# Illumina/Pisces

Measured on AMD Instinct MI355X. Metric: candidate loci/s at 500x depth, higher is better.
Workload: dtype int32 counts + f64 likelihoods; 1 GPU; BASELINE config 2: synthetic 100000 loci x 500x amplicon pileup, SNV-only, gVCF, per GPU per step; device-resident packed tuples; depth=500, ring_batches=6, tile_loci=56, parallelism=interval-shard x1

## Files before the change

### pisces_amd/build.py

```python
import os
import shutil
import subprocess

HERE = os.path.dirname(os.path.abspath(__file__))
CSRC = os.path.join(HERE, "csrc")
LIB = os.path.join(HERE, "libpisceship.so")
SOURCES = ["pisces_hip.hip", "expander.cpp", "finder.cpp", "vcf_format.cpp", "diploid.cpp"]
HEADERS = ["kernels.hip.h", "stream_kernels.hip.h", "store_kernels.hip.h", "surface_store.inc.h", "finder_kernels.hip.h", "bgzf_kernels.hip.h", "bam_kernels.hip.h", "device_math.hip.h", "surface_reads.inc.h", "surface_flush.inc.h", "surface_device.inc.h", "surface_bam.inc.h", "surface_comm.inc.h", "expander.h", "read_walk.h", "finder.h", "finder_walk.h", "diploid.h", "genotype_core.h", os.path.join("..", "..", "include", "pisces_hip.h")]


def hipcc_path():
    for cand in (shutil.which("hipcc"), "/opt/rocm/bin/hipcc"):
        if cand and os.path.exists(cand):
            return cand
    raise RuntimeError("hipcc not found (need ROCm: /opt/rocm/bin/hipcc)")


def is_stale():
    if not os.path.exists(LIB):
        return True
    t = os.path.getmtime(LIB)
    return any(os.path.getmtime(os.path.join(CSRC, f)) > t for f in SOURCES + HEADERS)


def source_hash():
    import hashlib
    hsh = hashlib.sha1()
    for f in sorted(SOURCES + HEADERS):
        with open(os.path.join(CSRC, f), "rb") as fp:
            hsh.update(f.encode() + b"\0" + fp.read())
    return hsh.hexdigest()


LAST_BUILD = {"mode": None, "seconds": 0.0}


def build_native(force=False, verbose=False, extra_flags=(), out=None):
    import time
    lib = LIB if out is None else out
    if out is None and not force and not is_stale():
        LAST_BUILD.update(mode="reused", seconds=0.0)
        return lib
    t0 = time.time()
    tmp = f"{lib}.{os.getpid()}.tmp"
    cmd = [hipcc_path(), "--offload-arch=gfx950", "-O3", "-std=c++17", "-fPIC", "-shared", "-ffp-contract=off",
           "-fno-fast-math", "-Wall", "-Wno-unused-function", "-x", "hip",
           *extra_flags, *[os.path.join(CSRC, s) for s in SOURCES], "-lpthread", "-ldl", "-o", tmp]
    if verbose:
        print(" ".join(cmd))
    subprocess.check_call(cmd)
    os.replace(tmp, lib)
    if out is None:
        LAST_BUILD.update(mode="rebuilt", seconds=time.time() - t0)
    return lib


if __name__ == "__main__":
    import sys
    build_native(force="--force" in sys.argv, verbose=True)
    print(LIB)
```

### pisces_amd/csrc/kernels.hip.h

```cpp
#pragma once
#include <hip/hip_runtime.h>
#include <stdint.h>

#include "device_math.hip.h"
#include "genotype_core.h"

namespace pisces {

constexpr int kBlock = 256;
constexpr int kTile = 64;
constexpr int kFolded = 18;
constexpr int kUnroll = 8;
constexpr int kSlotsPerTile = 4 * kTile;
#ifndef PISCES_TOTAL_SHARDS
#define PISCES_TOTAL_SHARDS 64
#endif
constexpr int kTotalShards = PISCES_TOTAL_SHARDS;
constexpr int kTotalStride = 16;
constexpr int kRefMargin = 32;
constexpr int kRefWin = kTile + 2 * kRefMargin;
constexpr int kWaveRows = 32;
constexpr int kWaveRow = kTile;
constexpr int kWaveRegion = kWaveRows * kWaveRow;
constexpr int kQLutLds = 128;
// ... 39 lines not shown
        u32x4 v[kUnroll];
#pragma unroll
        for (int u = 0; u < kUnroll; u++) {
            int64_t j = i + (int64_t)u * kBlock;
            v[u] = j < n4 ? __builtin_nontemporal_load(&p4[j]) : (u32x4){~0u, ~0u, ~0u, ~0u};
        }
#pragma unroll
        for (int u = 0; u < kUnroll; u++) {
            op(v[u].x); op(v[u].y); op(v[u].z); op(v[u].w);
        }
    }
    for (int64_t i = aend + tid; i < end; i += kBlock) op(tuples[i]);
}

__device__ __forceinline__ void copy_record(PiscesCalledAllele* dst, const PiscesCalledAllele* src)
{
    const unsigned long long sb = (unsigned long long)__double_as_longlong(src->strand_bias_score);
    uint4* dp = reinterpret_cast<uint4*>(dst);
    dp[0] = make_uint4((uint32_t)src->position, (uint32_t)src->total_coverage, (uint32_t)src->allele_support, (uint32_t)src->reference_support);
    dp[1] = make_uint4((uint32_t)src->num_no_calls, (uint32_t)src->coverage_by_dir[0], (uint32_t)src->coverage_by_dir[1], (uint32_t)src->coverage_by_dir[2]);
    dp[2] = make_uint4((uint32_t)src->support_by_dir[0], (uint32_t)src->support_by_dir[1], (uint32_t)src->support_by_dir[2], (uint32_t)src->variant_qscore);
    dp[3] = make_uint4((uint32_t)sb, (uint32_t)(sb >> 32), (uint32_t)(uint16_t)src->genotype_qscore | ((uint32_t)(uint16_t)src->noise_level << 16), (uint32_t)src->filter_bits | ((uint32_t)src->info << 16));
}

struct PointCounts {
    int cov[3], sup[3];
    int total, nocalls, refsup, support;
};

struct HistBlock {
    static __device__ __forceinline__ int idx(int a, int d, int l) { return (a * 3 + d) * kTile + l; }
};
struct HistWave {
    static __device__ __forceinline__ int idx(int a, int d, int l) { return (a * 4 + d) * kWaveRow + (int)PISCES_TUPLE_COLUMN(l, d); }
};

struct HistLinear {
    static __device__ __forceinline__ int idx(int a, int d, int l) { return (a * 4 + d) * kWaveRow + l; }
};

struct LocusCounts { int h[6][3]; };

template <typename H = HistBlock>
__device__ __forceinline__ LocusCounts load_counts(const int* hist, int l)
{
    LocusCounts lc;
// ... 342 lines not shown
__device__ __forceinline__ void stream_tuples_wave(const uint32_t* __restrict__ tuples, int64_t begin, int64_t end, int lane, int wid,
                                                   Op op, Pre pre)
{
    int64_t abegin = (begin + 3) & ~(int64_t)3;
    int64_t aend = end & ~(int64_t)3;
    if (abegin > aend) { abegin = end; aend = end; }
    const int tid = wid * 64 + lane;
    const u32x4* __restrict__ p4 = reinterpret_cast<const u32x4*>(tuples + abegin);
    const uint32_t n4 = (uint32_t)((aend - abegin) >> 2);
    constexpr uint32_t kBatch = 64u * kWaveUnroll;
    const uint32_t nb = (uint32_t)__builtin_amdgcn_readfirstlane((int)((n4 + kBatch - 1) / kBatch));
    u32x4 cur[kWaveUnroll], nxt[kWaveUnroll];
    auto load = [&](u32x4* v, uint32_t b) {
#pragma unroll
        for (int u = 0; u < kWaveUnroll; u++) {
            const uint32_t j = min(b * kBatch + (uint32_t)u * 64u + (uint32_t)lane, n4 - 1u);
            v[u] = __builtin_nontemporal_load(&p4[j]);
        }
    };
    auto consume = [&](const u32x4* v) {
#pragma unroll
        for (int u = 0; u < kWaveUnroll; u++) { op(v[u].x); op(v[u].y); op(v[u].z); op(v[u].w); }
    };
    const bool streams = (uint32_t)wid < nb;
    if (NW == 2) {
        if (streams) load(cur, (uint32_t)__builtin_amdgcn_readfirstlane(wid));
        __builtin_amdgcn_sched_barrier(0);
        pre();
    } else {
        pre();
        if (streams) load(cur, (uint32_t)__builtin_amdgcn_readfirstlane(wid));
    }
    for (int64_t i = begin + tid; i < abegin; i += 64 * NW) op(tuples[i]);
    if (streams) {
        uint32_t b = (uint32_t)__builtin_amdgcn_readfirstlane(wid);
        const uint32_t m = (nb - b + NW - 1) / NW;
        for (uint32_t p = (m - 1) / 2; p > 0; p--) {
            load(nxt, b + NW);
            __builtin_amdgcn_sched_barrier(0);
            consume(cur);
            __builtin_amdgcn_sched_barrier(0);
            load(cur, b + 2 * NW);
            __builtin_amdgcn_sched_barrier(0);
            consume(nxt);
            __builtin_amdgcn_sched_barrier(0);
            b += 2 * NW;
        }
        if (((m - 1) & 1u) != 0) {
            load(nxt, b + NW);
            __builtin_amdgcn_sched_barrier(0);
            consume(cur);
            __builtin_amdgcn_sched_barrier(0);
#pragma unroll
            for (int u = 0; u < kWaveUnroll; u++) cur[u] = nxt[u];
            b += NW;
        }
        if (b == nb - 1 && (n4 % kBatch)) {
#pragma unroll
            for (int u = 0; u < kWaveUnroll; u++)
                if (b * kBatch + (uint32_t)u * 64u + (uint32_t)lane >= n4) cur[u] = (u32x4){~0u, ~0u, ~0u, ~0u};
        }
        consume(cur);
    }
    for (int64_t i = aend + tid; i < end; i += 64 * NW) op(tuples[i]);
}

__device__ __forceinline__ void wave_lds_sync()
{
    __builtin_amdgcn_fence(__ATOMIC_SEQ_CST, "workgroup");
    __builtin_amdgcn_wave_barrier();
}

template <typename H = HistWave>
__device__ __forceinline__ uint32_t slow_alleles(const int* hist, const uint8_t* s_refwin, uint32_t slow, int l, int pos, int rt, int ref_rank,
                                                 const uint8_t* __restrict__ ref, int64_t win_lo, int64_t win_hi, PiscesCalledAllele* slots,
                                                 const DeviceParams& P)
{
    uint32_t called = 0;
    const int ref_a = (rt < 4) ? rt : PISCES_ALLELE_N;
#pragma unroll 1
    for (int k = 0; k < 5; k++) {
        if (!((slow >> k) & 1u)) continue;
        const bool isRef = k == 4;
        const int a = isRef ? ref_a : allele_of_rank(k);
        const LocusCounts lc = load_counts_wave<H>(hist, l);
        const PointCounts c = point_counts_of(lc, a, isRef, rt, 0);
        int vq = 0;
        if (c.support > 0 && c.total != 0) vq = poisson_qscore_out_of_line(c.support, c.total, P.err_q, P.max_vq, P.ln10);
        if (!isRef && vq < P.min_vq) continue;
        SbResult sb = {0.0, 0, 0, 0};
        if (c.support > 0) sb = strand_bias_out_of_line(c.cov, c.sup, P);
        PiscesCalledAllele r;
        (void)finish_allele<false>(c, pos, a, isRef, rt, vq, sb, ref, win_lo, win_hi, P, r, s_refwin, kRefMargin + l);
        copy_record(&slots[isRef ? ref_rank : k], &r);
        if (!isRef) called |= 1u << k;
    }
    return called;
}

template <int NW, typename H = HistWave>
__device__ __forceinline__ void call_phase_wave(const int* hist, const uint8_t* s_refwin, uint8_t* s_vmask, const PiscesTile& tile, const int t,
                                                const int l, const int wid, const uint8_t* __restrict__ ref, const int32_t ref_start,
                                                const int64_t ref_len, PiscesCalledAllele* __restrict__ records,
                                                PiscesTileResult* __restrict__ tile_results, const DeviceParams& P
#ifdef PISCES_TIMING
                                                , const long long tc0, const long long tc1
#endif
                                                )
{
    const int pos = tile.start_position + l;
    const uint8_t refb = s_refwin[kRefMargin + l];
    const bool in_ref = l < tile.n_loci && refb != 0;
    const int rt = in_ref ? allele_type_of_base(refb) : PISCES_ALLELE_N;
    const int64_t win_lo = (int64_t)ref_start - 1, win_hi = win_lo + ref_len;
    auto slot_of = [&](int k) { return records + ((int64_t)t * kSlotsPerTile + l * 4 + k); };
    const bool dirty = locus_is_dirty(P, pos);
    const LocusCounts lc = load_counts_wave<H>(hist, l);
    const bool ref_wave = wid == 0, var_wave = wid == NW - 1;
    if (P.folded_out && ref_wave && l < tile.n_loci) {
        const unsigned rel = (unsigned)(pos - P.folded_first);
        if (rel < (unsigned)P.folded_n) {
            int32_t* const dst = P.folded_out + (size_t)rel * PISCES_FOLDED_PER_LOCUS;
#pragma unroll
            for (int a = 0; a < 6; a++)
#pragma unroll
                for (int d = 0; d < 3; d++) dst[a * 3 + d] = lc.h[a][d];
        }
    }

    const bool tabs = tables_complete(P);
    auto fast_allele = [&](const PointCounts& c, int a, bool isRef, PiscesCalledAllele& rec) -> bool {
        int vq = 0;
        double sb_score = 0.0;
        int sb_ok = 0, sb_var = 0, sb_cov = 0;
        if (!tabs) return false;
        const AlleleTables tb = request_allele_tables(isRef, c.support, c.total, c.refsup, c.cov, c.sup, P);
        if (c.support > 0 && c.total != 0 && !poisson_qscore_try(c.support, c.total, P, tb, vq)) return false;
        if (!isRef && vq < P.min_vq) return true;
        if (c.support > 0 && !strand_bias_try(c.cov, c.sup, P, tb, sb_score, sb_ok, sb_var, sb_cov)) return false;
        const GqPre g = {tb.gq_idx, tb.gq_cap};
        const SbResult sb = {sb_score, sb_ok, sb_var, sb_cov};
        if (!finish_allele<true>(c, pos, a, isRef, rt, vq, sb, ref, win_lo, win_hi, P, rec, s_refwin, kRefMargin + l, nullptr, &g)) return false;
        return true;
    };
    bool ref_emitted = false;
    int ref_rank = 0;
    uint32_t slow = 0;
    uint32_t vmask = 0;
    const int ref_a = (rt < 4) ? rt : PISCES_ALLELE_N;
    if (ref_wave) {
        const PointCounts c = point_counts_of(lc, ref_a, true, rt, 0);
        if (in_ref && P.include_ref && !P.variants_only && (P.emit_zero_cov || c.total + c.nocalls > 0)) {
            ref_rank = (rt < 4) ? rank_of_allele(rt) : 0;
            ref_emitted = true;
            PiscesCalledAllele rec;
            if (fast_allele(c, ref_a, true, rec)) copy_record(slot_of(ref_rank), &rec);
            else slow |= 16u;
        }
    }
#ifdef PISCES_TIMING
    const long long tcA = wall_clock64();
#endif
    if (var_wave && in_ref && rt < 4 && !P.refs_only && !dirty) {
#pragma unroll 1
        for (int k = 0; k < 4; k++) {
            const int a = allele_of_rank(k);
            if (a == rt) continue;
            const PointCounts c = point_counts_of(lc, a, false, rt, 0);
            if (c.support == 0) continue;
            if (!variant_passes_frequency(c, P)) continue;
            PiscesCalledAllele r;
            r.position = 0;
            if (!fast_allele(c, a, false, r)) { slow |= 1u << k; continue; }
            if (r.position == 0) continue;
            copy_record(slot_of(k), &r);
            vmask |= 1u << k;
        }
    }
    if (__builtin_expect(__ballot(slow != 0) != 0ull, 0))
        vmask |= slow_alleles<H>(hist, s_refwin, slow, l, pos, rt, ref_rank, ref, win_lo, win_hi, records + ((int64_t)t * kSlotsPerTile + l * 4), P);
    if (NW == 2) {
        if (var_wave) s_vmask[l] = (uint8_t)vmask;
        __syncthreads();
        if (!ref_wave) return;
        vmask = s_vmask[l];
    }
#ifdef PISCES_TIMING
    const long long tcB = wall_clock64();
#endif

    const uint32_t valid = vmask ? vmask : (ref_emitted ? (1u << ref_rank) : 0u);
    int n_surv = 0, n_var = 0;
#pragma unroll
    for (int k = 0; k < 4; k++) {
        n_surv += __popcll(__ballot((valid >> k) & 1u));
        n_var += __popcll(__ballot((vmask >> k) & 1u));
    }
    const int n_call_total = n_var + __popcll(__ballot(ref_emitted));
    const int n_loci_called = __popcll(__ballot(valid != 0));
    uint32_t word = valid << ((l & 7) * 4);
    word |= __shfl_xor(word, 1, 64);
    word |= __shfl_xor(word, 2, 64);
    word |= __shfl_xor(word, 4, 64);
// ... 7 lines not shown
        if (P.totals) {
            unsigned long long* tt = P.totals + (size_t)(t % kTotalShards) * kTotalStride;
            atomicAdd(&tt[0], (unsigned long long)n_surv);
            atomicAdd(&tt[1], (unsigned long long)n_loci_called);
            atomicAdd(&tt[2], (unsigned long long)n_call_total);
            atomicAdd(&tt[3], 1ull);
        }
#ifdef PISCES_TIMING
        const long long tc2 = wall_clock64();
        tile_result->record_begin = (int)(tc0 & 0x3FFFFFFF);
        tile_result->n_records = (int)(tc1 & 0x3FFFFFFF);
        tile_result->n_candidate_loci = (int)(tc2 & 0x3FFFFFFF);
        tile_result->n_called = (int)__builtin_amdgcn_s_getreg(63492);
        tile_result->valid[0] = __builtin_amdgcn_s_getreg(63508);
        tile_result->valid[1] = 0;
        tile_result->valid[2] = (uint32_t)(tcA - tc1);
        tile_result->valid[3] = (uint32_t)(tcB - tcA);
        tile_result->valid[4] = 0;
        tile_result->valid[5] = (uint32_t)(tc2 - tcB);
#endif
    }
}

template <int NW>
__global__ __launch_bounds__(64 * NW, NW == 1 ? PISCES_WAVE_OCC : PISCES_WAVE2_OCC) void call_tiles_wave_kernel(
    const uint32_t* __restrict__ tuples, const PiscesTile* __restrict__ tiles, int32_t n_tiles,
    const uint8_t* __restrict__ ref, int32_t ref_start, int64_t ref_len, PiscesCalledAllele* __restrict__ records,
    PiscesTileResult* __restrict__ tile_results, DeviceParams P, const DeviceParams* __restrict__ Pd )
{
    __shared__ __attribute__((aligned(16))) int hist[2 * kWaveRegion];
    __shared__ uint8_t s_refwin[kRefWin];
    __shared__ uint8_t s_vmask[kTile];

    const int t = blockIdx.x;
    if (t >= n_tiles) return;
    const int l = threadIdx.x & 63, wid = threadIdx.x >> 6;
    const PiscesTile tile = tiles[t];
#ifdef PISCES_TIMING
    const long long tc0 = wall_clock64();
#endif
    auto setup = [&]() {
        int4* h4 = reinterpret_cast<int4*>(hist);
        for (int i = threadIdx.x; i < 2 * kWaveRegion / 4; i += 64 * NW) h4[i] = make_int4(0, 0, 0, 0);
        for (int i = threadIdx.x; i < kRefWin; i += 64 * NW) {
            const int64_t ri = (int64_t)tile.start_position - kRefMargin + i - ref_start;
            s_refwin[i] = (ri >= 0 && ri < ref_len) ? ref[ri] : (uint8_t)0;
        }
        __syncthreads();
    };

    {
        if (NW == 2) __builtin_amdgcn_s_setprio(3);
        const uint32_t min_bq_shifted = (uint32_t)min(max(P.min_bq, 0), 255) << 24;
        stream_tuples_wave<NW>(tuples, tile.tuple_begin, tile.tuple_end, l, wid, [&](uint32_t v) { accumulate_wave(hist, v, min_bq_shifted); }, setup);
    }
    __syncthreads();
    if (NW == 2) __builtin_amdgcn_s_setprio(0);
#ifdef PISCES_TIMING
    const long long tc1 = wall_clock64();
#endif

    call_phase_wave<NW>(hist, s_refwin, s_vmask, tile, t, l, wid, ref, ref_start, ref_len, records, tile_results, P
#ifdef PISCES_TIMING
                        , tc0, tc1
#endif
                        );
}

__global__ __launch_bounds__(256) void build_vq_tab_kernel(int16_t* __restrict__ tab, int32_t n_k, int32_t n_cov, DeviceParams P)
{
    const int64_t i = (int64_t)blockIdx.x * blockDim.x + threadIdx.x;
    if (i >= (int64_t)n_k * n_cov) return;
    tab[i] = (int16_t)poisson_qscore((int32_t)(i / n_cov), (int32_t)(i % n_cov), P);
}
__global__ __launch_bounds__(256) void build_sb_tab_kernel(double* __restrict__ tab, double* __restrict__ tab0, int32_t n_k, int32_t n_cov, DeviceParams P)
{
    const int64_t i = (int64_t)blockIdx.x * blockDim.x + threadIdx.x;
    if (i >= (int64_t)n_k * n_cov) return;
    const int k = (int)(i / n_cov), cov = (int)(i % n_cov);
    tab[i] = k >= 1 ? fmax(0.0, poisson_cdf_sb((double)k - 1, (double)cov * P.err_sb)) : 0.0;
    if (k == 0) tab0[cov] = pow(1 - P.err_sb, (double)cov);
}
__global__ __launch_bounds__(256) void build_gq_cap_kernel(int16_t* __restrict__ tab, const double* __restrict__ gq_tail, int32_t n_a, int32_t n_cov, DeviceParams P)
{
    const int64_t i = (int64_t)blockIdx.x * blockDim.x + threadIdx.x;
// ... 830 lines not shown
```

### pisces_amd/csrc/pisces_hip.hip

```cpp
#include <hip/hip_runtime.h>
#include <hip/hip_ext.h>
#include <dlfcn.h>
#include <link.h>

#include <algorithm>
#include <array>
#include <cctype>
#include <memory>
#include <cmath>
#include <cstdio>
#include <cstdlib>
#include <cstring>
#include <deque>
#include <ctime>
#include <map>
#include <set>
#include <string>
#include <atomic>
#include <chrono>
#include <mutex>
#include <thread>
#include <unordered_map>
#include <unordered_set>
#include <vector>
// ... 255 lines not shown
    int32_t* h_cnt_x = nullptr;
    bool tables_shareable = false;
    bool poisoned = false;
    std::string poison_why;
    uint8_t* h_prep = nullptr;
    DeviceBuf<double> d_qlut;
    DeviceBuf<ulonglong2> d_bq_lut;
    DeviceBuf<unsigned long long> d_sumq_fix;
    DeviceBuf<double> d_sumq;
    DeviceBuf<double> d_gq_tail;
    DeviceBuf<int16_t> d_vq_tab;
    DeviceBuf<double> d_sb_tab;
    DeviceBuf<double> d_sb0_tab;
    DeviceBuf<int16_t> d_gq_cap;
    DeviceBuf<DeviceParams> d_params;
    int n_cus = 256;
    void* comm = nullptr;
    int comm_world = 1;
    DeviceBuf<long long> d_summary;
    DeviceBuf<int32_t> d_offsets;
    DeviceBuf<PiscesCalledAllele> d_compact;
    DeviceBuf<PiscesGenotypePosteriors> d_post, d_post_compact;
    int kernel_variant = 4;
    std::string err;

    DeviceBuf<uint8_t> d_ref;
    std::vector<uint8_t> h_ref;
    int64_t ref_len = 0;
    DeviceBuf<DevCandidate> d_cands;
    DeviceBuf<uint8_t> d_alleles;
    DeviceBuf<PiscesCalledAllele> d_cand_records;
    DeviceBuf<uint8_t> d_cand_callable;
    int32_t* h_counts = nullptr;
    size_t h_counts_cap = 0;

    std::map<int32_t, BlockObs> blocks;
    int32_t last_block_key_cache = 0;
    BlockObs* last_block = nullptr;
    int32_t last_up_to_block_key = 0;
    std::unordered_map<int32_t, int32_t> gapped_mnv_ref;
    std::vector<HostCandidate> known_variants;
    bool exclude_mnvs_from_collapsing = false;
    std::vector<HostCandidate> forced;
    size_t n_forced_added = 0;
    std::set<std::string> forced_keys;
    std::set<int32_t> forced_positions;
// ... 468 lines not shown
    h->device = device;
    if ((e = hipSetDevice(device)) != hipSuccess || (e = hipStreamCreateWithFlags(&h->stream, hipStreamNonBlocking)) != hipSuccess ||
        (e = hipEventCreate(&h->ev0)) != hipSuccess || (e = hipEventCreate(&h->ev1)) != hipSuccess) {
        g_create_error = std::string("pisces_hip_create: ") + hipGetErrorString(e);
        delete h;
        return PISCES_E_DEVICE;
    }
    if ((e = h->d_totals.reserve((size_t)kTotalShards * kTotalStride)) != hipSuccess ||
        (e = hipMemsetAsync(h->d_totals.p, 0, (size_t)kTotalShards * kTotalStride * sizeof(unsigned long long), h->stream)) != hipSuccess ||
        (e = hipStreamSynchronize(h->stream)) != hipSuccess) {
        g_create_error = std::string("pisces_hip_create: ") + hipGetErrorString(e);
        pisces_hip_destroy(h);
        return PISCES_E_DEVICE;
    }
    h->P.totals = h->d_totals.p;
    {
        hipDeviceProp_t prop;
        if (hipGetDeviceProperties(&prop, device) == hipSuccess && prop.multiProcessorCount > 0) h->n_cus = prop.multiProcessorCount;
        const char* kv = getenv("PISCES_HIP_KERNEL");
        if (kv && std::string(kv) == "wave") h->kernel_variant = 2;
        if (kv && std::string(kv) == "wave2") h->kernel_variant = 3;
        if (kv && std::string(kv) == "auto") h->kernel_variant = 4;
        if (kv && std::string(kv) == "block") h->kernel_variant = 0;
        h->prof_on = getenv("PISCES_HIP_HOST_PROFILE") != nullptr;
        const char* rp = getenv("PISCES_HIP_READ_PATH");
        if (rp && std::string(rp) == "log") h->read_path = 0;
        if (const char* v = getenv("PISCES_HIP_STORE_DIRECT_BYTES")) h->store_direct_bytes = (size_t)std::max(0ll, atoll(v));
        if (const char* v = getenv("PISCES_HIP_STORE_WAVES")) h->store_waves = atoi(v);
        if (const char* v = getenv("PISCES_HIP_TILE_ORDER")) h->trade_tiles = atoi(v) != 0;
        if (const char* v = getenv("PISCES_HIP_DEVICE_MERGE")) h->device_merge = atoi(v) != 0 ? 1 : 0;
        h->snv_walk = h->cfg.call_mnvs != 0 || (h->cfg.collapse != 0 && (h->cfg.collapse_freq_threshold > 0.0f || h->cfg.collapse_freq_ratio_threshold >= 1.0f));
        h->mnv_split = h->snv_walk && h->device_merge != 0;
        if (const char* v = getenv("PISCES_HIP_MNV_SPLIT")) h->mnv_split = h->mnv_split && atoi(v) != 0;
        if (const char* v = getenv("PISCES_HIP_STORE_SEAL_BYTES")) h->store_seal_bytes = (size_t)std::max(0ll, atoll(v));
        if (const char* v = getenv("PISCES_HIP_DEVICE_CHECKS")) h->device_checks = atoi(v) != 0 ? 1 : 0;
        if (const char* v = getenv("PISCES_HIP_TILE_LOCI")) h->tile_loci = atoi(v);
        if (const char* v = getenv("PISCES_HIP_DEFER_GRID")) h->defer_grid = atoi(v) != 0;
        if (const char* v = getenv("PISCES_HIP_COMPACT")) h->compact_mode = std::string(v) == "two" ? 2 : std::string(v) == "lookback" ? 3 : 0;
        if (const char* v = getenv("PISCES_HIP_MERGE_IN_PLACE")) h->merge_in_place = atoi(v) != 0;
        if (const char* v = getenv("PISCES_HIP_DEVICE_GENOTYPER")) h->device_genotyper = atoi(v) != 0;
        if (const char* v = getenv("PISCES_HIP_FINDER")) h->finder_bases = std::string(v) == "bases";
    }
    {
        const int n = std::min(std::max(h->cfg.max_variant_qscore, 0), 4095) + 1;
        std::vector<double> lut((size_t)n);
        for (int q = 0; q < n; q++) lut[(size_t)q] = std::pow(10.0, -1 * (double)q / 10.0);
// ... 294 lines not shown
```

### pisces_amd/csrc/surface_device.inc.h

```cpp

int32_t pisces_hip_call_tiles(PiscesHip* h, const uint32_t* d_tuples, const PiscesTile* d_tiles, int32_t n_tiles,
                              const uint8_t* d_ref_bases, int32_t ref_start_position, int64_t ref_length,
                              PiscesCalledAllele* d_records, int32_t record_capacity, PiscesTileResult* d_tile_results, void* stream)
{
    return abi_guard<int32_t>(h, [&]() -> int32_t {
    if (!h) return PISCES_E_INVALID_ARG;
    if (n_tiles < 0 || record_capacity < 0 || ref_length < 0) return fail(h, PISCES_E_INVALID_ARG, "call_tiles: negative size");
    if (n_tiles > 0 && (!d_tiles || !d_ref_bases || !d_records || !d_tile_results))
        return fail(h, PISCES_E_INVALID_ARG, "call_tiles: null device pointer");
    if ((int64_t)record_capacity < (int64_t)n_tiles * kSlotsPerTile)
        return fail(h, PISCES_E_BUFFER_TOO_SMALL, "call_tiles: the slot layout needs record_capacity >= 256 * n_tiles");
    if (h->d_posteriors && h->posteriors_capacity < (int64_t)n_tiles * kSlotsPerTile)
        return fail(h, PISCES_E_BUFFER_TOO_SMALL, "call_tiles: the posteriors buffer (pisces_hip_set_posteriors_buffer) needs 256 * n_tiles entries");
    PISCES_HIP_CHECK(h, hipSetDevice(h->device));
    hipStream_t s = stream ? (hipStream_t)stream : h->stream;
    if (s != h->stream) h->foreign_stream_used = h->foreign_stream_ever = true;
    hipEvent_t e0 = nullptr, e1 = nullptr;
    if (h->timing > 0 && (h->launches_seen++ % h->timing) == 0) {
        const size_t slot = (size_t)(h->ring_used % kTimingRing);
        e0 = h->ring[2 * slot];
        e1 = h->ring[2 * slot + 1];
        h->ring_used++;
    }
    if (n_tiles > 0) {
        PISCES_HIP_CHECK(h, launch_call_tiles(h, s, d_tuples, d_tiles, n_tiles, d_ref_bases, ref_start_position, ref_length, d_records, d_tile_results, e0, e1));
        if (germline(h)) launch_genotype_loci(h, s, d_records, d_tile_results, n_tiles, h->d_posteriors);
    } else if (e0) {
        PISCES_HIP_CHECK(h, hipEventRecord(e0, s));
        PISCES_HIP_CHECK(h, hipEventRecord(e1, s));
    }
    PISCES_HIP_CHECK(h, hipGetLastError());
    return PISCES_OK;
    });
}

int32_t pisces_hip_balanced_tile_loci(PiscesHip* h, int64_t n_loci)
{
    return abi_guard<int32_t>(h, [&]() -> int32_t {
    if (!h || n_loci <= 0) return kTile;
    const int64_t cus = std::max(1, h->n_cus);
    const int64_t per_cu = (n_loci + (int64_t)kTile * cus - 1) / ((int64_t)kTile * cus);
    if (per_cu > 8) return kTile;
    const int64_t n_tiles = per_cu * cus;
    return (int32_t)std::min<int64_t>(kTile, (n_loci + n_tiles - 1) / n_tiles);
    });
}

int32_t pisces_hip_call_tiles_batched(PiscesHip* h, const PiscesTileBatch* batches, int32_t n_batches, void* stream)
// ... 3 lines not shown
    if (n_batches < 0 || (n_batches > 0 && !batches)) return fail(h, PISCES_E_INVALID_ARG, "call_tiles_batched: null batch list");
    if (h->cfg.ploidy == PISCES_PLOIDY_DIPLOID_ADAPTIVE)
        return fail(h, PISCES_E_UNSUPPORTED, "call_tiles_batched: PloidyModel.DiploidByAdaptiveGT has one posteriors buffer a handle; use pisces_hip_call_tiles");
    if (h->cfg.noise_model == PISCES_NOISE_WINDOW)
        return fail(h, PISCES_E_STATE, "call_tiles_batched: NoiseModel.Window calls through the handle's one counts tensor; use pisces_hip_call_tiles");
    for (int32_t i = 0; i < n_batches; i++) {
        const PiscesTileBatch& b = batches[i];
        if (b.n_tiles < 0 || b.record_capacity < 0 || b.ref_length < 0) return fail(h, PISCES_E_INVALID_ARG, "call_tiles: negative size");
        if (b.n_tiles > 0 && (!b.d_tiles || !b.d_ref_bases || !b.d_records || !b.d_tile_results))
            return fail(h, PISCES_E_INVALID_ARG, "call_tiles: null device pointer");
        if ((int64_t)b.record_capacity < (int64_t)b.n_tiles * kSlotsPerTile)
            return fail(h, PISCES_E_BUFFER_TOO_SMALL, "call_tiles: the slot layout needs record_capacity >= 256 * n_tiles");
    }
    if (n_batches == 0) return PISCES_OK;
    PISCES_HIP_CHECK(h, hipSetDevice(h->device));
    if (!h->lane[0])
        for (int k = 0; k < PiscesHip::kLanes; k++) PISCES_HIP_CHECK(h, hipStreamCreateWithFlags(&h->lane[k], hipStreamNonBlocking));
    const int lanes = std::min<int>(PiscesHip::kLanes, n_batches);
    if (stream) PISCES_HIP_CHECK(h, hipStreamSynchronize((hipStream_t)stream));
    for (int32_t i = 0; i < n_batches; i++) {
        const PiscesTileBatch& b = batches[i];
        if (b.n_tiles == 0) continue;
        PISCES_HIP_CHECK(h, launch_call_tiles(h, h->lane[i % lanes], b.d_tuples, b.d_tiles, b.n_tiles, b.d_ref_bases, b.ref_start_position,
                                              b.ref_length, b.d_records, b.d_tile_results));
        if (germline(h)) launch_genotype_loci(h, h->lane[i % lanes], b.d_records, b.d_tile_results, b.n_tiles);
    }
    PISCES_HIP_CHECK(h, hipGetLastError());
    return PISCES_OK;
    });
}

int32_t pisces_hip_call_tiles_graph_build(PiscesHip* h, const PiscesTileBatch* batches, int32_t n_batches, int32_t* graph_id)
{
    return abi_guard<int32_t>(h, [&]() -> int32_t {
    if (!h || !graph_id) return PISCES_E_INVALID_ARG;
    if (n_batches <= 0 || !batches) return fail(h, PISCES_E_INVALID_ARG, "call_tiles_graph_build: null batch list");
    if (h->cfg.ploidy == PISCES_PLOIDY_DIPLOID_ADAPTIVE)
        return fail(h, PISCES_E_UNSUPPORTED, "call_tiles_graph_build: PloidyModel.DiploidByAdaptiveGT has one posteriors buffer a handle; use pisces_hip_call_tiles");
    if (h->cfg.noise_model == PISCES_NOISE_WINDOW)
        return fail(h, PISCES_E_STATE, "call_tiles_graph_build: NoiseModel.Flat only (see pisces_hip_call_tiles_batched)");
    for (int32_t i = 0; i < n_batches; i++) {
        const PiscesTileBatch& b = batches[i];
        if (b.n_tiles <= 0 || b.record_capacity < 0 || b.ref_length < 0 || !b.d_tiles || !b.d_ref_bases || !b.d_records || !b.d_tile_results)
            return fail(h, PISCES_E_INVALID_ARG, "call_tiles_graph_build: bad batch");
        if ((int64_t)b.record_capacity < (int64_t)b.n_tiles * kSlotsPerTile)
            return fail(h, PISCES_E_BUFFER_TOO_SMALL, "call_tiles: the slot layout needs record_capacity >= 256 * n_tiles");
    }
    PISCES_HIP_CHECK(h, hipSetDevice(h->device));
    PISCES_HIP_CHECK(h, hipStreamSynchronize(h->stream));
    hipGraph_t graph = nullptr;
    PISCES_HIP_CHECK(h, hipStreamBeginCapture(h->stream, hipStreamCaptureModeThreadLocal));
    hipError_t e = hipSuccess;
    for (int32_t i = 0; i < n_batches && e == hipSuccess; i++) {
        const PiscesTileBatch& b = batches[i];
        hipEvent_t e0 = nullptr, e1 = nullptr;
        if (h->timing > 0 && (h->launches_seen++ % h->timing) == 0 && h->ring_used < kTimingRing) {
            const size_t slot = (size_t)h->ring_used;
            e0 = h->ring[2 * slot];
            e1 = h->ring[2 * slot + 1];
            h->ring_used++;
        }
        if (e0) e = hipEventRecord(e0, h->stream);
        if (e == hipSuccess)
            e = launch_call_tiles(h, h->stream, b.d_tuples, b.d_tiles, b.n_tiles, b.d_ref_bases, b.ref_start_position, b.ref_length, b.d_records,
                                  b.d_tile_results);
        if (e == hipSuccess && germline(h)) launch_genotype_loci(h, h->stream, b.d_records, b.d_tile_results, b.n_tiles);
        if (e == hipSuccess && e1) e = hipEventRecord(e1, h->stream);
    }
    const hipError_t ec = hipStreamEndCapture(h->stream, &graph);
    if (e == hipSuccess) e = ec;
    if (e == hipSuccess) e = hipGetLastError();
    hipGraphExec_t exec = nullptr;
    if (e == hipSuccess) e = hipGraphInstantiate(&exec, graph, nullptr, nullptr, 0);
    if (e != hipSuccess) {
        if (graph) (void)hipGraphDestroy(graph);
        return fail(h, PISCES_E_DEVICE, std::string("call_tiles_graph_build: ") + hipGetErrorString(e));
    }
    if (hipGraphUpload(exec, h->stream) == hipSuccess) (void)hipStreamSynchronize(h->stream);
    else (void)hipGetLastError();
    h->graph_defs.push_back(graph);
    h->graphs.push_back(exec);
    *graph_id = (int32_t)h->graphs.size() - 1;
    return PISCES_OK;
    });
}

int32_t pisces_hip_call_tiles_graph_launch(PiscesHip* h, int32_t graph_id, void* stream)
{
// ... 242 lines not shown
```

### pisces_amd/csrc/surface_flush.inc.h

```cpp

static void tile_geometry(PiscesHip* h, const std::vector<int32_t>& keys, bool clip, std::vector<PiscesTile>& tiles,
                          std::vector<int32_t>& first_tile, std::vector<int32_t>& tol)
{
    tiles.clear();
    first_tile.clear();
    tol.clear();
    const int bs = h->cfg.block_size;
    const bool irregular = clip && !h->intervals.empty();
    if (irregular) tol.assign(keys.size() * (size_t)bs, -1);
    for (size_t ki = 0; ki < keys.size(); ki++) {
        const int32_t key = keys[ki];
        const int32_t bstart = (key - 1) * bs + 1, bend = key * bs;
        const size_t first = tiles.size();
        first_tile.push_back((int32_t)first);
        auto add_range = [&](int32_t s, int32_t e) {
            for (int32_t p = s; p <= e; p += kTile) {
                PiscesTile t;
                t.start_position = p;
                t.n_loci = std::min<int32_t>(kTile, e - p + 1);
                t.tuple_begin = t.tuple_end = 0;
                if (irregular)
                    for (int32_t q = 0; q < t.n_loci; q++) tol[ki * (size_t)bs + (size_t)(p + q - bstart)] = (int32_t)(tiles.size() - first);
                tiles.push_back(t);
            }
// ... 100 lines not shown
    PISCES_HIP_CHECK(h, hipGetLastError());
    return PISCES_OK;
}
static void commit_drop(PiscesHip* h, unsigned long long kept)
{
    h->log_cur ^= 1;
    h->log_ub = (int64_t)kept;
    h->log_known_holes = 0;
}
static int32_t drop_blocks(PiscesHip* h, const std::vector<int32_t>& keys)
{
    if (keys.empty() || h->log_ub == 0) return PISCES_OK;
    int32_t rc = enqueue_drop(h, keys);
    if (rc) return rc;
    unsigned long long kept = 0;
    PISCES_HIP_CHECK(h, hipMemcpyAsync(&kept, h->d_log_n.p + (h->log_cur ^ 1), sizeof(kept), hipMemcpyDeviceToHost, h->stream));
    PISCES_HIP_CHECK(h, hipStreamSynchronize(h->stream));
    commit_drop(h, kept);
    return PISCES_OK;
}

static hipError_t launch_call_tiles(PiscesHip* h, hipStream_t s, const uint32_t* d_tuples, const PiscesTile* d_tiles, int32_t n_tiles,
                              const uint8_t* d_ref, int32_t ref_start, int64_t ref_len, PiscesCalledAllele* d_records,
                              PiscesTileResult* d_tr, hipEvent_t e0 = nullptr, hipEvent_t e1 = nullptr)
{
    if (h->cfg.noise_model == PISCES_NOISE_WINDOW) {
        if (e0) (void)hipEventRecord(e0, s);
        hipError_t er = accumulate_tiles(h, s, d_tuples, d_tiles, n_tiles, true);
        if (er != hipSuccess) return er;
        hipLaunchKernelGGL(call_counts_kernel, dim3((unsigned)n_tiles), dim3(kBlock), 0, s, h->d_counts.p, (const uint32_t*)nullptr, d_tiles, n_tiles,
                           d_ref, ref_start, ref_len, d_records, d_tr, h->P, h->d_sumq.p);
        if (e1) (void)hipEventRecord(e1, s);
        return hipSuccess;
    }
    if (h->kernel_variant >= 2 && h->cfg.min_base_call_quality <= 255 && h->cfg.strand_bias_model != PISCES_SB_DIPLOID) {
        const bool two = h->kernel_variant == 3 || (h->kernel_variant == 4 && (int64_t)n_tiles <= (int64_t)h->n_cus * 32);
        if (!two && !e0 && !e1)
            hipLaunchKernelGGL(call_tiles_wave_kernel<1>, dim3((unsigned)n_tiles), dim3(64), 0, s, d_tuples, d_tiles, n_tiles, d_ref, ref_start, ref_len,
                               d_records, d_tr, h->P, (const DeviceParams*)h->d_params.p);
        else if (!two)
            hipExtLaunchKernelGGL(call_tiles_wave_kernel<1>, dim3((unsigned)n_tiles), dim3(64), 0, s, e0, e1, 0u, d_tuples, d_tiles,
                                  n_tiles, d_ref, ref_start, ref_len, d_records, d_tr, h->P, (const DeviceParams*)h->d_params.p);
        else if (!e0 && !e1)
            hipLaunchKernelGGL(call_tiles_wave_kernel<2>, dim3((unsigned)n_tiles), dim3(128), 0, s, d_tuples, d_tiles, n_tiles, d_ref, ref_start, ref_len,
                               d_records, d_tr, h->P, (const DeviceParams*)h->d_params.p);
        else
            hipExtLaunchKernelGGL(call_tiles_wave_kernel<2>, dim3((unsigned)n_tiles), dim3(128), 0, s, e0, e1, 0u, d_tuples, d_tiles,
                                  n_tiles, d_ref, ref_start, ref_len, d_records, d_tr, h->P, (const DeviceParams*)h->d_params.p);
        return hipSuccess;
    }
    hipExtLaunchKernelGGL(call_tiles_kernel, dim3((unsigned)n_tiles), dim3(kBlock), 0, s, e0, e1, 0u, d_tuples, d_tiles, n_tiles, d_ref,
                          ref_start, ref_len, d_records, d_tr, h->P);
    return hipSuccess;
}

static void launch_genotype_loci(PiscesHip* h, hipStream_t s, PiscesCalledAllele* d_records, PiscesTileResult* d_tr, int32_t n_tiles,
                                 PiscesGenotypePosteriors* d_posteriors = nullptr)
{
    GenotypeParams G;
    G.ploidy = h->cfg.ploidy;
    for (int k = 0; k < 3; k++) { G.snv[k] = h->cfg.diploid_snv_params[k]; G.indel[k] = h->cfg.diploid_indel_params[k]; }
    G.min_depth = h->cfg.min_coverage;
    G.min_gq = h->cfg.min_genotype_qscore;
    G.max_gq = h->cfg.max_genotype_qscore;
    G.low_gq_filter = h->cfg.low_gq_filter;
    if (n_tiles <= 0) return;
    if (h->cfg.ploidy == PISCES_PLOIDY_DIPLOID_ADAPTIVE)
        hipLaunchKernelGGL(genotype_loci_adaptive_kernel, dim3((unsigned)n_tiles), dim3(64), 0, s, d_records, d_tr, n_tiles, G, h->adaptive, d_posteriors, h->P.totals);
    else hipLaunchKernelGGL(genotype_loci_kernel, dim3((unsigned)n_tiles), dim3(64), 0, s, d_records, d_tr, n_tiles, G, h->P.totals);
}
static bool germline(const PiscesHip* h)
{
    return h->cfg.ploidy == PISCES_PLOIDY_DIPLOID || h->cfg.ploidy == PISCES_PLOIDY_HAPLOID || h->cfg.ploidy == PISCES_PLOIDY_DIPLOID_ADAPTIVE;
}

static int32_t launch_compaction(PiscesHip* h, hipStream_t s, const PiscesCalledAllele* d_records, const PiscesTileResult* d_tr, int32_t n_tiles,
                                 int32_t* d_offsets, PiscesCalledAllele* d_out, int32_t cap, int32_t* d_count, int32_t* d_called = nullptr)
{
    if (h->compact_mode == 2 || (n_tiles > kGatherDirectTiles && s != h->stream)) {
        hipLaunchKernelGGL(scan_tile_counts_kernel, dim3(1), dim3(1024), 0, s, d_tr, n_tiles, d_offsets, d_count, d_called);
        hipLaunchKernelGGL(gather_records_kernel, dim3((unsigned)n_tiles), dim3(64), 0, s, d_records, d_tr, n_tiles, d_offsets, d_out, cap);
        return PISCES_OK;
    }
    if (n_tiles <= kGatherDirectTiles && h->compact_mode != 3) {
        hipLaunchKernelGGL(gather_direct_kernel, dim3((unsigned)n_tiles), dim3(64), 0, s, d_records, d_tr, n_tiles, d_offsets, d_out, cap, d_count, d_called);
        return PISCES_OK;
    }
    const size_t groups = ((size_t)n_tiles + kCompactTiles - 1) / kCompactTiles;
    {
        const size_t before = h->d_compact_state.cap;
        PISCES_HIP_CHECK(h, h->d_compact_state.reserve(groups));
        if (h->d_compact_state.cap != before || h->compact_epoch >= (1u << 30) - 1u) {
            PISCES_HIP_CHECK(h, hipMemsetAsync(h->d_compact_state.p, 0, h->d_compact_state.cap * sizeof(unsigned long long), s));
            h->compact_epoch = 0;
        }
    }
    const uint32_t epoch = ++h->compact_epoch;
// ... 2383 lines not shown
```

Baseline: 2.560 billion candidate loci/s.

## Deepen two-wave tuple prefetch and add write-through buffer stores for records

In the two-wave call kernel, the tuple stream now issues two batches of loads before the histogram setup runs and keeps two batches in flight throughout the main loop. The last-batch masking is factored into a helper. Each thread also fetches its reference-window byte before setup, and a compiler barrier pins the kernel arguments in scalar registers. Record slot writes can now go through raw buffer stores with a write-through cache policy, enabled by default for non-germline runs and selectable by an environment variable. The aim is to hide global load latency behind setup and cut cache pollution from record stores, at the cost of more live registers and another kernel template variant.

```diff
diff --git a/pisces_amd/build.py b/pisces_amd/build.py
--- a/pisces_amd/build.py
+++ b/pisces_amd/build.py
@@ -32,6 +32,8 @@
     return hsh.hexdigest()
 
 
+COMPILE_FLAGS = ["--offload-arch=gfx950", "-O3", "-std=c++17", "-fPIC", "-ffp-contract=off", "-fno-fast-math", "-Wall", "-Wno-unused-function"]
+
 LAST_BUILD = {"mode": None, "seconds": 0.0}
 
 
@@ -43,8 +45,7 @@
         return lib
     t0 = time.time()
     tmp = f"{lib}.{os.getpid()}.tmp"
-    cmd = [hipcc_path(), "--offload-arch=gfx950", "-O3", "-std=c++17", "-fPIC", "-shared", "-ffp-contract=off",
-           "-fno-fast-math", "-Wall", "-Wno-unused-function", "-x", "hip",
+    cmd = [hipcc_path(), *COMPILE_FLAGS, "-shared", "-x", "hip",
            *extra_flags, *[os.path.join(CSRC, s) for s in SOURCES], "-lpthread", "-ldl", "-o", tmp]
     if verbose:
         print(" ".join(cmd))
diff --git a/pisces_amd/csrc/kernels.hip.h b/pisces_amd/csrc/kernels.hip.h
--- a/pisces_amd/csrc/kernels.hip.h
+++ b/pisces_amd/csrc/kernels.hip.h
@@ -85,6 +85,34 @@
     dp[2] = make_uint4((uint32_t)src->support_by_dir[0], (uint32_t)src->support_by_dir[1], (uint32_t)src->support_by_dir[2], (uint32_t)src->variant_qscore);
     dp[3] = make_uint4((uint32_t)sb, (uint32_t)(sb >> 32), (uint32_t)(uint16_t)src->genotype_qscore | ((uint32_t)(uint16_t)src->noise_level << 16), (uint32_t)src->filter_bits | ((uint32_t)src->info << 16));
 }
+
+template <bool WT> struct TileSlots;
+template <> struct TileSlots<false> {
+    PiscesCalledAllele* base;
+    __device__ __forceinline__ TileSlots(PiscesCalledAllele* records, int t) : base(records + (int64_t)t * kSlotsPerTile) {}
+    __device__ __forceinline__ void store(int slot, const PiscesCalledAllele& r) const { copy_record(base + slot, &r); }
+};
+template <> struct TileSlots<true> {
+    __amdgpu_buffer_rsrc_t rsrc;
+    static constexpr int kRawBufferWord3 = 0x00020000;
+    static constexpr int kWriteThrough = 16;
+    __device__ __forceinline__ TileSlots(PiscesCalledAllele* records, int t)
+        : rsrc(__builtin_amdgcn_make_buffer_rsrc(records + (int64_t)t * kSlotsPerTile, 0, kSlotsPerTile * (int)sizeof(PiscesCalledAllele), kRawBufferWord3)) {}
+    __device__ __forceinline__ void store(int slot, const PiscesCalledAllele& r) const
+    {
+        const unsigned long long sb = (unsigned long long)__double_as_longlong(r.strand_bias_score);
+        const int off = slot * (int)sizeof(PiscesCalledAllele);
+        const u32x4 w0 = {(uint32_t)r.position, (uint32_t)r.total_coverage, (uint32_t)r.allele_support, (uint32_t)r.reference_support};
+        const u32x4 w1 = {(uint32_t)r.num_no_calls, (uint32_t)r.coverage_by_dir[0], (uint32_t)r.coverage_by_dir[1], (uint32_t)r.coverage_by_dir[2]};
+        const u32x4 w2 = {(uint32_t)r.support_by_dir[0], (uint32_t)r.support_by_dir[1], (uint32_t)r.support_by_dir[2], (uint32_t)r.variant_qscore};
+        const u32x4 w3 = {(uint32_t)sb, (uint32_t)(sb >> 32), (uint32_t)(uint16_t)r.genotype_qscore | ((uint32_t)(uint16_t)r.noise_level << 16),
+                          (uint32_t)r.filter_bits | ((uint32_t)r.info << 16)};
+        __builtin_amdgcn_raw_buffer_store_b128(w0, rsrc, off, 0, kWriteThrough);
+        __builtin_amdgcn_raw_buffer_store_b128(w1, rsrc, off + 16, 0, kWriteThrough);
+        __builtin_amdgcn_raw_buffer_store_b128(w2, rsrc, off + 32, 0, kWriteThrough);
+        __builtin_amdgcn_raw_buffer_store_b128(w3, rsrc, off + 48, 0, kWriteThrough);
+    }
+};
 
 struct PointCounts {
     int cov[3], sup[3];
@@ -473,15 +501,60 @@
 #pragma unroll
         for (int u = 0; u < kWaveUnroll; u++) { op(v[u].x); op(v[u].y); op(v[u].z); op(v[u].w); }
     };
+    auto mask_last = [&](u32x4* v, uint32_t b) {
+        if (b == nb - 1 && (n4 % kBatch)) {
+#pragma unroll
+            for (int u = 0; u < kWaveUnroll; u++)
+                if (b * kBatch + (uint32_t)u * 64u + (uint32_t)lane >= n4) v[u] = (u32x4){~0u, ~0u, ~0u, ~0u};
+        }
+    };
     const bool streams = (uint32_t)wid < nb;
     if (NW == 2) {
-        if (streams) load(cur, (uint32_t)__builtin_amdgcn_readfirstlane(wid));
-        __builtin_amdgcn_sched_barrier(0);
-        pre();
-    } else {
-        pre();
-        if (streams) load(cur, (uint32_t)__builtin_amdgcn_readfirstlane(wid));
-    }
+        uint32_t b = (uint32_t)__builtin_amdgcn_readfirstlane(wid);
+        const uint32_t m = b < nb ? (nb - b + NW - 1) / NW : 0u;
+        if (__builtin_expect(m >= 2, 1)) {
+            load(cur, b);
+            load(nxt, b + NW);
+            __builtin_amdgcn_sched_barrier(0);
+            pre();
+            for (uint32_t p = (m - 2) / 2; p > 0; p--) {
+                consume(cur);
+                __builtin_amdgcn_sched_barrier(0);
+                load(cur, b + 2 * NW);
+                __builtin_amdgcn_sched_barrier(0);
+                consume(nxt);
+                __builtin_amdgcn_sched_barrier(0);
+                load(nxt, b + 3 * NW);
+                __builtin_amdgcn_sched_barrier(0);
+                b += 2 * NW;
+            }
+            consume(cur);
+            __builtin_amdgcn_sched_barrier(0);
+            if ((m & 1u) != 0) {
+                load(cur, b + 2 * NW);
+                __builtin_amdgcn_sched_barrier(0);
+                consume(nxt);
+                mask_last(cur, b + 2 * NW);
+                consume(cur);
+            } else {
+                mask_last(nxt, b + NW);
+                consume(nxt);
+            }
+        } else {
+            if (m == 1) load(cur, b);
+            __builtin_amdgcn_sched_barrier(0);
+            pre();
+            if (m == 1) {
+                mask_last(cur, b);
+                consume(cur);
+            }
+        }
+        for (int64_t i = begin + tid; i < abegin; i += 64 * NW) op(tuples[i]);
+        for (int64_t i = aend + tid; i < end; i += 64 * NW) op(tuples[i]);
+        return;
+    }
+    pre();
+    if (streams) load(cur, (uint32_t)__builtin_amdgcn_readfirstlane(wid));
     for (int64_t i = begin + tid; i < abegin; i += 64 * NW) op(tuples[i]);
     if (streams) {
         uint32_t b = (uint32_t)__builtin_amdgcn_readfirstlane(wid);
@@ -506,11 +579,7 @@
             for (int u = 0; u < kWaveUnroll; u++) cur[u] = nxt[u];
             b += NW;
         }
-        if (b == nb - 1 && (n4 % kBatch)) {
-#pragma unroll
-            for (int u = 0; u < kWaveUnroll; u++)
-                if (b * kBatch + (uint32_t)u * 64u + (uint32_t)lane >= n4) cur[u] = (u32x4){~0u, ~0u, ~0u, ~0u};
-        }
+        mask_last(cur, b);
         consume(cur);
     }
     for (int64_t i = aend + tid; i < end; i += 64 * NW) op(tuples[i]);
@@ -522,9 +591,9 @@
     __builtin_amdgcn_wave_barrier();
 }
 
-template <typename H = HistWave>
+template <typename H = HistWave, bool WT = false>
 __device__ __forceinline__ uint32_t slow_alleles(const int* hist, const uint8_t* s_refwin, uint32_t slow, int l, int pos, int rt, int ref_rank,
-                                                 const uint8_t* __restrict__ ref, int64_t win_lo, int64_t win_hi, PiscesCalledAllele* slots,
+                                                 const uint8_t* __restrict__ ref, int64_t win_lo, int64_t win_hi, const TileSlots<WT>& slots,
                                                  const DeviceParams& P)
 {
     uint32_t called = 0;
@@ -543,13 +612,13 @@
         if (c.support > 0) sb = strand_bias_out_of_line(c.cov, c.sup, P);
         PiscesCalledAllele r;
         (void)finish_allele<false>(c, pos, a, isRef, rt, vq, sb, ref, win_lo, win_hi, P, r, s_refwin, kRefMargin + l);
-        copy_record(&slots[isRef ? ref_rank : k], &r);
+        slots.store(l * 4 + (isRef ? ref_rank : k), r);
         if (!isRef) called |= 1u << k;
     }
     return called;
 }
 
-template <int NW, typename H = HistWave>
+template <int NW, typename H = HistWave, bool WT = false>
 __device__ __forceinline__ void call_phase_wave(const int* hist, const uint8_t* s_refwin, uint8_t* s_vmask, const PiscesTile& tile, const int t,
                                                 const int l, const int wid, const uint8_t* __restrict__ ref, const int32_t ref_start,
                                                 const int64_t ref_len, PiscesCalledAllele* __restrict__ records,
@@ -564,7 +633,7 @@
     const bool in_ref = l < tile.n_loci && refb != 0;
     const int rt = in_ref ? allele_type_of_base(refb) : PISCES_ALLELE_N;
     const int64_t win_lo = (int64_t)ref_start - 1, win_hi = win_lo + ref_len;
-    auto slot_of = [&](int k) { return records + ((int64_t)t * kSlotsPerTile + l * 4 + k); };
+    const TileSlots<WT> slots(records, t);
     const bool dirty = locus_is_dirty(P, pos);
     const LocusCounts lc = load_counts_wave<H>(hist, l);
     const bool ref_wave = wid == 0, var_wave = wid == NW - 1;
@@ -605,7 +674,7 @@
             ref_rank = (rt < 4) ? rank_of_allele(rt) : 0;
             ref_emitted = true;
             PiscesCalledAllele rec;
-            if (fast_allele(c, ref_a, true, rec)) copy_record(slot_of(ref_rank), &rec);
+            if (fast_allele(c, ref_a, true, rec)) slots.store(l * 4 + ref_rank, rec);
             else slow |= 16u;
         }
     }
@@ -624,12 +693,12 @@
             r.position = 0;
             if (!fast_allele(c, a, false, r)) { slow |= 1u << k; continue; }
             if (r.position == 0) continue;
-            copy_record(slot_of(k), &r);
+            slots.store(l * 4 + k, r);
             vmask |= 1u << k;
         }
     }
     if (__builtin_expect(__ballot(slow != 0) != 0ull, 0))
-        vmask |= slow_alleles<H>(hist, s_refwin, slow, l, pos, rt, ref_rank, ref, win_lo, win_hi, records + ((int64_t)t * kSlotsPerTile + l * 4), P);
+        vmask |= slow_alleles<H, WT>(hist, s_refwin, slow, l, pos, rt, ref_rank, ref, win_lo, win_hi, slots, P);
     if (NW == 2) {
         if (var_wave) s_vmask[l] = (uint8_t)vmask;
         __syncthreads();
@@ -683,7 +752,7 @@
     }
 }
 
-template <int NW>
+template <int NW, bool WT>
 __global__ __launch_bounds__(64 * NW, NW == 1 ? PISCES_WAVE_OCC : PISCES_WAVE2_OCC) void call_tiles_wave_kernel(
     const uint32_t* __restrict__ tuples, const PiscesTile* __restrict__ tiles, int32_t n_tiles,
     const uint8_t* __restrict__ ref, int32_t ref_start, int64_t ref_len, PiscesCalledAllele* __restrict__ records,
@@ -694,19 +763,30 @@
     __shared__ uint8_t s_vmask[kTile];
 
     const int t = blockIdx.x;
-    if (t >= n_tiles) return;
+    int32_t n_tiles_ = n_tiles;
+    asm("" : "+s"(n_tiles_) : "s"(tuples), "s"(tiles), "s"(ref), "s"(ref_start), "s"(ref_len));
+    if (t >= n_tiles_) return;
     const int l = threadIdx.x & 63, wid = threadIdx.x >> 6;
     const PiscesTile tile = tiles[t];
 #ifdef PISCES_TIMING
     const long long tc0 = wall_clock64();
 #endif
+    auto ref_byte = [&](int i) -> uint8_t {
+        const int64_t ri = (int64_t)tile.start_position - kRefMargin + i - ref_start;
+        return (ri >= 0 && ri < ref_len) ? ref[ri] : (uint8_t)0;
+    };
+    static_assert(NW != 2 || kRefWin == 64 * NW, "one reference byte a thread");
+    uint8_t my_ref = 0;
+    if (NW == 2) {
+        my_ref = ref_byte(threadIdx.x);
+        __builtin_amdgcn_sched_barrier(0);
+    }
     auto setup = [&]() {
         int4* h4 = reinterpret_cast<int4*>(hist);
         for (int i = threadIdx.x; i < 2 * kWaveRegion / 4; i += 64 * NW) h4[i] = make_int4(0, 0, 0, 0);
-        for (int i = threadIdx.x; i < kRefWin; i += 64 * NW) {
-            const int64_t ri = (int64_t)tile.start_position - kRefMargin + i - ref_start;
-            s_refwin[i] = (ri >= 0 && ri < ref_len) ? ref[ri] : (uint8_t)0;
-        }
+        if (NW == 2) s_refwin[threadIdx.x] = my_ref;
+        else
+            for (int i = threadIdx.x; i < kRefWin; i += 64 * NW) s_refwin[i] = ref_byte(i);
         __syncthreads();
     };
 
@@ -721,7 +801,7 @@
     const long long tc1 = wall_clock64();
 #endif
 
-    call_phase_wave<NW>(hist, s_refwin, s_vmask, tile, t, l, wid, ref, ref_start, ref_len, records, tile_results, P
+    call_phase_wave<NW, HistWave, WT>(hist, s_refwin, s_vmask, tile, t, l, wid, ref, ref_start, ref_len, records, tile_results, P
 #ifdef PISCES_TIMING
                         , tc0, tc1
 #endif
diff --git a/pisces_amd/csrc/pisces_hip.hip b/pisces_amd/csrc/pisces_hip.hip
--- a/pisces_amd/csrc/pisces_hip.hip
+++ b/pisces_amd/csrc/pisces_hip.hip
@@ -301,6 +301,7 @@
     DeviceBuf<PiscesCalledAllele> d_compact;
     DeviceBuf<PiscesGenotypePosteriors> d_post, d_post_compact;
     int kernel_variant = 4;
+    bool records_through = true;
     std::string err;
 
     DeviceBuf<uint8_t> d_ref;
@@ -815,6 +816,7 @@
         if (kv && std::string(kv) == "wave2") h->kernel_variant = 3;
         if (kv && std::string(kv) == "auto") h->kernel_variant = 4;
         if (kv && std::string(kv) == "block") h->kernel_variant = 0;
+        if (const char* v = getenv("PISCES_HIP_RECORD_STORES")) h->records_through = std::string(v) != "plain";
         h->prof_on = getenv("PISCES_HIP_HOST_PROFILE") != nullptr;
         const char* rp = getenv("PISCES_HIP_READ_PATH");
         if (rp && std::string(rp) == "log") h->read_path = 0;
diff --git a/pisces_amd/csrc/surface_device.inc.h b/pisces_amd/csrc/surface_device.inc.h
--- a/pisces_amd/csrc/surface_device.inc.h
+++ b/pisces_amd/csrc/surface_device.inc.h
@@ -23,7 +23,8 @@
         h->ring_used++;
     }
     if (n_tiles > 0) {
-        PISCES_HIP_CHECK(h, launch_call_tiles(h, s, d_tuples, d_tiles, n_tiles, d_ref_bases, ref_start_position, ref_length, d_records, d_tile_results, e0, e1));
+        PISCES_HIP_CHECK(h, launch_call_tiles(h, s, d_tuples, d_tiles, n_tiles, d_ref_bases, ref_start_position, ref_length, d_records, d_tile_results, e0, e1,
+                                              records_written_through(h)));
         if (germline(h)) launch_genotype_loci(h, s, d_records, d_tile_results, n_tiles, h->d_posteriors);
     } else if (e0) {
         PISCES_HIP_CHECK(h, hipEventRecord(e0, s));
@@ -73,7 +74,7 @@
         const PiscesTileBatch& b = batches[i];
         if (b.n_tiles == 0) continue;
         PISCES_HIP_CHECK(h, launch_call_tiles(h, h->lane[i % lanes], b.d_tuples, b.d_tiles, b.n_tiles, b.d_ref_bases, b.ref_start_position,
-                                              b.ref_length, b.d_records, b.d_tile_results));
+                                              b.ref_length, b.d_records, b.d_tile_results, nullptr, nullptr, records_written_through(h)));
         if (germline(h)) launch_genotype_loci(h, h->lane[i % lanes], b.d_records, b.d_tile_results, b.n_tiles);
     }
     PISCES_HIP_CHECK(h, hipGetLastError());
@@ -114,7 +115,7 @@
         if (e0) e = hipEventRecord(e0, h->stream);
         if (e == hipSuccess)
             e = launch_call_tiles(h, h->stream, b.d_tuples, b.d_tiles, b.n_tiles, b.d_ref_bases, b.ref_start_position, b.ref_length, b.d_records,
-                                  b.d_tile_results);
+                                  b.d_tile_results, nullptr, nullptr, records_written_through(h));
         if (e == hipSuccess && germline(h)) launch_genotype_loci(h, h->stream, b.d_records, b.d_tile_results, b.n_tiles);
         if (e == hipSuccess && e1) e = hipEventRecord(e1, h->stream);
     }
diff --git a/pisces_amd/csrc/surface_flush.inc.h b/pisces_amd/csrc/surface_flush.inc.h
--- a/pisces_amd/csrc/surface_flush.inc.h
+++ b/pisces_amd/csrc/surface_flush.inc.h
@@ -146,7 +146,7 @@
 
 static hipError_t launch_call_tiles(PiscesHip* h, hipStream_t s, const uint32_t* d_tuples, const PiscesTile* d_tiles, int32_t n_tiles,
                               const uint8_t* d_ref, int32_t ref_start, int64_t ref_len, PiscesCalledAllele* d_records,
-                              PiscesTileResult* d_tr, hipEvent_t e0 = nullptr, hipEvent_t e1 = nullptr)
+                              PiscesTileResult* d_tr, hipEvent_t e0 = nullptr, hipEvent_t e1 = nullptr, bool write_through = false)
 {
     if (h->cfg.noise_model == PISCES_NOISE_WINDOW) {
         if (e0) (void)hipEventRecord(e0, s);
@@ -159,18 +159,18 @@
     }
     if (h->kernel_variant >= 2 && h->cfg.min_base_call_quality <= 255 && h->cfg.strand_bias_model != PISCES_SB_DIPLOID) {
         const bool two = h->kernel_variant == 3 || (h->kernel_variant == 4 && (int64_t)n_tiles <= (int64_t)h->n_cus * 32);
-        if (!two && !e0 && !e1)
-            hipLaunchKernelGGL(call_tiles_wave_kernel<1>, dim3((unsigned)n_tiles), dim3(64), 0, s, d_tuples, d_tiles, n_tiles, d_ref, ref_start, ref_len,
-                               d_records, d_tr, h->P, (const DeviceParams*)h->d_params.p);
-        else if (!two)
-            hipExtLaunchKernelGGL(call_tiles_wave_kernel<1>, dim3((unsigned)n_tiles), dim3(64), 0, s, e0, e1, 0u, d_tuples, d_tiles,
-                                  n_tiles, d_ref, ref_start, ref_len, d_records, d_tr, h->P, (const DeviceParams*)h->d_params.p);
-        else if (!e0 && !e1)
-            hipLaunchKernelGGL(call_tiles_wave_kernel<2>, dim3((unsigned)n_tiles), dim3(128), 0, s, d_tuples, d_tiles, n_tiles, d_ref, ref_start, ref_len,
-                               d_records, d_tr, h->P, (const DeviceParams*)h->d_params.p);
-        else
-            hipExtLaunchKernelGGL(call_tiles_wave_kernel<2>, dim3((unsigned)n_tiles), dim3(128), 0, s, e0, e1, 0u, d_tuples, d_tiles,
-                                  n_tiles, d_ref, ref_start, ref_len, d_records, d_tr, h->P, (const DeviceParams*)h->d_params.p);
+        auto launch = [&](auto kernel, unsigned block) {
+            if (!e0 && !e1)
+                hipLaunchKernelGGL(kernel, dim3((unsigned)n_tiles), dim3(block), 0, s, d_tuples, d_tiles, n_tiles, d_ref, ref_start, ref_len, d_records, d_tr,
+                                   h->P, (const DeviceParams*)h->d_params.p);
+            else
+                hipExtLaunchKernelGGL(kernel, dim3((unsigned)n_tiles), dim3(block), 0, s, e0, e1, 0u, d_tuples, d_tiles, n_tiles, d_ref, ref_start, ref_len,
+                                      d_records, d_tr, h->P, (const DeviceParams*)h->d_params.p);
+        };
+        if (!two && !write_through) launch(call_tiles_wave_kernel<1, false>, 64u);
+        else if (!two) launch(call_tiles_wave_kernel<1, true>, 64u);
+        else if (!write_through) launch(call_tiles_wave_kernel<2, false>, 128u);
+        else launch(call_tiles_wave_kernel<2, true>, 128u);
         return hipSuccess;
     }
     hipExtLaunchKernelGGL(call_tiles_kernel, dim3((unsigned)n_tiles), dim3(kBlock), 0, s, e0, e1, 0u, d_tuples, d_tiles, n_tiles, d_ref,
@@ -197,6 +197,8 @@
 {
     return h->cfg.ploidy == PISCES_PLOIDY_DIPLOID || h->cfg.ploidy == PISCES_PLOIDY_HAPLOID || h->cfg.ploidy == PISCES_PLOIDY_DIPLOID_ADAPTIVE;
 }
+
+static bool records_written_through(const PiscesHip* h) { return h->records_through && !germline(h); }
 
 static int32_t launch_compaction(PiscesHip* h, hipStream_t s, const PiscesCalledAllele* d_records, const PiscesTileResult* d_tr, int32_t n_tiles,
                                  int32_t* d_offsets, PiscesCalledAllele* d_out, int32_t cap, int32_t* d_count, int32_t* d_called = nullptr)
```

Result: slower. 2.356 billion candidate loci/s (-8.0%).
